# CelestineAngla/BundleAdjustment.jl

Hardware: AMD Instinct MI355X
Metric: LM iterations/sec on BAL venice-1778 (synthetic BAL-shaped), plus Jacobian Mnnz/sec (higher is better)
Workload: dtype f64; 1 GPU; venice-1778 shape: ncams=1778 npnts=993923 nobs=5001946, seed 20261004, lm.jl variant, LDL/None, facto_type f64, fixed 83 iterations, perm AMD; parallelism=points sharded over 1 rank(s), cameras replicated

## Files before the change

bundleadjustment.jl_amd/csrc/ba_dense_ldl.hip:

```cpp
#include "ba_internal.h"

#include <algorithm>
#include <atomic>
#include <cmath>
#include <cstdio>
#include <cstdlib>

namespace {

template <typename T>
struct RT;
template <>
struct RT<double> {
  typedef double v4 __attribute__((ext_vector_type(4)));
  typedef double v2 __attribute__((ext_vector_type(2)));
  static __device__ inline v4 mfma(double a, double b, v4 c) { return __builtin_amdgcn_mfma_f64_16x16x4f64(a, b, c, 0, 0, 0); }
  static __device__ inline int row(int lane, int reg) { return (lane >> 4) + 4 * reg; }
};
template <>
struct RT<float> {
  typedef float v4 __attribute__((ext_vector_type(4)));
  typedef float v2 __attribute__((ext_vector_type(2)));
  static __device__ inline v4 mfma(float a, float b, v4 c) { return __builtin_amdgcn_mfma_f32_16x16x4f32(a, b, c, 0, 0, 0); }
  static __device__ inline int row(int lane, int reg) { return 4 * (lane >> 4) + reg; }
// ... 1272 lines not shown
  matvec_t(Linv + (int64_t)k * NB * NB, zk);
  __syncthreads();
  if (tid < NB) xk[tid] = part[0][tid] + part[1][tid];
  __syncthreads();
  if (tkk >= 0) matvec_t(S + tkk * NB * NB, xk);
  else part[half][c] = 0;
  __syncthreads();
  if (tid < NB) {
    const T d = D[(int64_t)(k - 1) * NB + tid];
    zk[tid] = (y[(int64_t)(k - 1) * NB + tid] - d * (part[0][tid] + part[1][tid])) / d;
  }
  __syncthreads();
  matvec_t(Linv + (int64_t)(k - 1) * NB * NB, zk);
  __syncthreads();
  if (tid < NB) xk1[tid] = part[0][tid] + part[1][tid];
  __syncthreads();
  if (bid == 0) {
    if (tid < NB) {
      x[(int64_t)k * NB + tid] = xk[tid];
      x[(int64_t)(k - 1) * NB + tid] = xk1[tid];
    }
    return;
  }
  const T *Lkj = S + tkj * NB * NB, *Lk1j = S + tk1j * NB * NB;
  T s = 0;
  if (tkj >= 0 && tk1j >= 0) {
    for (int r = half * 64; r < half * 64 + 64; r++) s += Lkj[r * NB + c] * xk[r] + Lk1j[r * NB + c] * xk1[r];
  } else if (tkj >= 0) {
    for (int r = half * 64; r < half * 64 + 64; r++) s += Lkj[r * NB + c] * xk[r];
  } else if (tk1j >= 0) {
    for (int r = half * 64; r < half * 64 + 64; r++) s += Lk1j[r * NB + c] * xk1[r];
  }
  part[half][c] = s;
  __syncthreads();
  if (tid < NB) y[(int64_t)j * NB + tid] -= D[(int64_t)j * NB + tid] * (part[0][tid] + part[1][tid]);
}

template <typename T>
__global__ __launch_bounds__(256) void k_bwd_pair(const T *__restrict__ S, const int64_t *__restrict__ co, const T *__restrict__ Linv,
                                                   const T *__restrict__ D, T *__restrict__ y, T *__restrict__ x, int k,
                                                   const int *__restrict__ cols = nullptr) {
  bwd_pair_body<T>(S, co, Linv, D, y, x, k, cols, (int)blockIdx.x);
}
template <typename T>
__global__ __launch_bounds__(256) void k_bwd_pair2(const T *__restrict__ S, const int64_t *__restrict__ co, const T *__restrict__ Linv,
                                                    const T *__restrict__ D, T *__restrict__ y, T *__restrict__ x, int ka,
                                                    const int *__restrict__ cols_a, int na, int kc, const int *__restrict__ cols_c) {
  const bool second = (int)blockIdx.x >= na;
  bwd_pair_body<T>(S, co, Linv, D, y, x, second ? kc : ka, second ? cols_c : cols_a, (int)blockIdx.x - (second ? na : 0));
}


template <typename T>
__global__ __launch_bounds__(256) void k_fwd_step_multi(const T *__restrict__ S, const int64_t *__restrict__ co, const T *__restrict__ Linv,
                                                         T *__restrict__ b, T *__restrict__ y, int k, int64_t ld) {
  BA_VT
  __shared__ T yk[NB];
  const int tid = threadIdx.x, lane = tid & 63, wv = tid >> 6;
  const int i = k + blockIdx.x;
  const int64_t tik = blockIdx.x == 0 ? 0 : tix(co, i, k);
  if (tik < 0) return;
  b += (int64_t)blockIdx.y * ld;
  y += (int64_t)blockIdx.y * ld;
  const T *Lk = Linv + (int64_t)k * NB * NB;
  const d2 bk = *reinterpret_cast<const d2 *>(b + (int64_t)k * NB + 2 * lane);
  for (int rr = 0; rr < 32; rr++) {
    int row = wv * 32 + rr;
    d2 l = *reinterpret_cast<const d2 *>(Lk + row * NB + 2 * lane);
    T s = wsum(l.x * bk.x + l.y * bk.y);
    if (lane == 0) yk[row] = s;
  }
  __syncthreads();
  if (blockIdx.x == 0) {
    if (tid < NB) y[(int64_t)k * NB + tid] = yk[tid];
    return;
  }
  const T *Lik = S + tik * NB * NB;
  const T y0 = yk[2 * lane], y1 = yk[2 * lane + 1];
  for (int rr = 0; rr < 32; rr++) {
    int row = wv * 32 + rr;
    d2 l = *reinterpret_cast<const d2 *>(Lik + row * NB + 2 * lane);
    T s = wsum(l.x * y0 + l.y * y1);
    if (lane == 0) b[(int64_t)i * NB + row] -= s;
  }
}

template <typename T>
__global__ __launch_bounds__(256) void k_bwd_step_multi(const T *__restrict__ S, const int64_t *__restrict__ co, const T *__restrict__ Linv,
                                                         const T *__restrict__ D, T *__restrict__ y, T *__restrict__ x, int k, int64_t ld) {
  __shared__ T zk[NB], xk[NB], part[2][NB];
  const int tid = threadIdx.x;
  const int c = tid & (NB - 1), half = tid >> 7;
  const int j = (int)blockIdx.x - 1;
  const int64_t tkj = blockIdx.x == 0 ? 0 : tix(co, k, j);
  if (tkj < 0) return;
  y += (int64_t)blockIdx.y * ld;
  x += (int64_t)blockIdx.y * ld;
  if (tid < NB) zk[tid] = y[(int64_t)k * NB + tid] / D[(int64_t)k * NB + tid];
  __syncthreads();
  {
    const T *Lk = Linv + (int64_t)k * NB * NB;
    T s = 0;
    for (int r = half * 64; r < half * 64 + 64; r++) s += Lk[r * NB + c] * zk[r];
    part[half][c] = s;
  }
  __syncthreads();
  if (tid < NB) xk[tid] = part[0][tid] + part[1][tid];
  __syncthreads();
  if (blockIdx.x == 0) {
    if (tid < NB) x[(int64_t)k * NB + tid] = xk[tid];
    return;
  }
  const T *Lkj = S + tkj * NB * NB;
  T s = 0;
  for (int r = half * 64; r < half * 64 + 64; r++) s += Lkj[r * NB + c] * xk[r];
  part[half][c] = s;
  __syncthreads();
  if (tid < NB) y[(int64_t)j * NB + tid] -= D[(int64_t)j * NB + tid] * (part[0][tid] + part[1][tid]);
}

}

int64_t dense_ldl_tiles_doubles(int64_t n_unpadded) {
  int64_t nt = (n_unpadded + NB - 1) / NB;
  if (nt < 1) nt = 1;
  return nt * (nt + 1) / 2 * NB * NB;
}

template <typename T>
static int set_kernel_attrs() {
  static std::atomic<bool> g_attr_done{false};
  if (g_attr_done.load()) return BA_OK;
  BA_HIP_CHECK(hipFuncSetAttribute(reinterpret_cast<const void *>(k_ldl_diag<T>),
                                   hipFuncAttributeMaxDynamicSharedMemorySize, (int)(DIAG_LDS_ELEMS * sizeof(T))));
  BA_HIP_CHECK(hipFuncSetAttribute(reinterpret_cast<const void *>(k_ldl_update<T, 1>),
                                   hipFuncAttributeMaxDynamicSharedMemorySize, (int)gemm_priv_lds_bytes<T>()));
  BA_HIP_CHECK(hipFuncSetAttribute(reinterpret_cast<const void *>(k_ldl_pairdiag<T, true>),
                                   hipFuncAttributeMaxDynamicSharedMemorySize, (int)(DIAG_LDS_ELEMS * sizeof(T))));
  BA_HIP_CHECK(hipFuncSetAttribute(reinterpret_cast<const void *>(k_ldl_pairdiag<T, false>),
                                   hipFuncAttributeMaxDynamicSharedMemorySize, (int)(DIAG_LDS_ELEMS * sizeof(T))));
  BA_HIP_CHECK(hipFuncSetAttribute(reinterpret_cast<const void *>(k_ldl_pairtrsm<T, true>),
                                   hipFuncAttributeMaxDynamicSharedMemorySize, (int)(PT_LDS_ELEMS * sizeof(T))));
  BA_HIP_CHECK(hipFuncSetAttribute(reinterpret_cast<const void *>(k_ldl_pairtrsm<T, false>),
                                   hipFuncAttributeMaxDynamicSharedMemorySize, (int)(PT_LDS_ELEMS * sizeof(T))));
  BA_HIP_CHECK(hipFuncSetAttribute(reinterpret_cast<const void *>(k_ldl_update_rs<T>),
                                   hipFuncAttributeMaxDynamicSharedMemorySize, (int)(RS_LDS_ELEMS * sizeof(T))));
  BA_HIP_CHECK(hipFuncSetAttribute(reinterpret_cast<const void *>(k_ldl_update2<T>), hipFuncAttributeMaxDynamicSharedMemorySize,
                                   (int)gemm_priv_lds_bytes<T>()));
  BA_HIP_CHECK(hipFuncSetAttribute(reinterpret_cast<const void *>(k_ldl_diag2<T>), hipFuncAttributeMaxDynamicSharedMemorySize,
                                   (int)(DIAG_LDS_ELEMS * sizeof(T))));
  BA_HIP_CHECK(hipFuncSetAttribute(reinterpret_cast<const void *>(k_ldl_update_part2<T>), hipFuncAttributeMaxDynamicSharedMemorySize,
                                   (int)part_lds_bytes<T>()));
  BA_HIP_CHECK(hipFuncSetAttribute(reinterpret_cast<const void *>(k_ldl_update_part<T>),
                                   hipFuncAttributeMaxDynamicSharedMemorySize, (int)part_lds_bytes<T>()));
  BA_HIP_CHECK(hipFuncSetAttribute(reinterpret_cast<const void *>(k_ldl_update<T, 1, true>),
                                   hipFuncAttributeMaxDynamicSharedMemorySize, (int)gemm_priv_lds_bytes<T>()));
  g_attr_done.store(true);
  return BA_OK;
}

void dense_ldl_layout(int64_t nt, int world, std::vector<int64_t> *col_off, std::vector<int64_t> *own_range) {
  col_off->assign((size_t)nt, 0);
  if (own_range) own_range->assign((size_t)world + 1, 0);
  int64_t off = 0;
  for (int r = 0; r < world; r++) {
    if (own_range) (*own_range)[(size_t)r] = off;
    for (int64_t q = r; 2 * q < nt; q += world)
      for (int64_t j = 2 * q; j < 2 * q + 2 && j < nt; j++) {
        (*col_off)[(size_t)j] = off;
        off += nt - j;
      }
  }
  if (own_range) (*own_range)[(size_t)world] = off;
}

template <typename T>
int dense_ldl_alloc(DenseLDLT<T> *w, int64_t n_unpadded, int world, int rank, bool lazy_S, bool own_only) {
  int64_t nt = (n_unpadded + NB - 1) / NB;
  if (nt < 1) nt = 1;
  w->n = nt * NB;
  w->nt = nt;
  w->world = world;
  w->rank = rank;
  dense_ldl_layout(nt, world, &w->h_glob_off, &w->own_range);
  w->h_col_tab.assign((size_t)nt + 1, 0);
  for (int64_t j = 0; j < nt; j++) w->hco()[j] = w->h_glob_off[(size_t)j];
  w->own_only = own_only && world > 1;
  w->s_tiles = nt * (nt + 1) / 2;
  if (w->own_only) {
    const int64_t base = w->own_range[(size_t)rank];
    for (int64_t j = 0; j < nt; j++)
      w->hco()[j] = ((j / 2) % world == rank) ? w->hco()[j] - base : BA_NO_TILE;
    w->s_tiles = std::max<int64_t>(1, w->own_range[(size_t)rank + 1] - base);
  }
  BA_CHECK(upload(w->col_tab, w->h_col_tab));
  w->col_off = w->col_tab + 1;
  w->h_own_cols.clear();
  w->h_own_pref.assign(1, 0);
  for (int64_t j = 0; j < nt; j++)
    if ((j / 2) % world == rank) {
      w->h_own_cols.push_back((int)j);
      w->h_own_pref.push_back(w->h_own_pref.back() + (nt - j));
    }
  BA_CHECK(upload(w->own_cols, w->h_own_cols, 1));
  BA_CHECK(upload(w->own_pref, w->h_own_pref));
  BA_CHECK(w->flag_sum.alloc(1));
  if (!lazy_S) BA_CHECK(dense_ldl_alloc_S(w));
  BA_CHECK(w->ev_chain.create(hipEventDisableTiming | hipEventReleaseToDevice));
  BA_CHECK(w->Linv.alloc(nt * NB * NB));
  BA_HIP_CHECK(hipMemset(w->Linv, 0, (size_t)nt * NB * NB * sizeof(T)));
  BA_HIP_CHECK(hipDeviceSynchronize());
  BA_CHECK(w->D.alloc(nt * NB * 2));
  BA_CHECK(w->flag.alloc(1));
  BA_CHECK(w->ready.alloc(nt));
  BA_CHECK(w->hoist.create(hipStreamNonBlocking));
  {
    int lo = 0, hi = 0;
    BA_HIP_CHECK(hipDeviceGetStreamPriorityRange(&lo, &hi));
    BA_CHECK(w->rest.create(hipStreamNonBlocking, lo));
  }
  BA_CHECK(w->ev_top.create(hipEventDisableTiming | hipEventReleaseToDevice));
  BA_CHECK(w->ev_dtop.create(hipEventDisableTiming));
  BA_CHECK(w->ev_dchain.create(hipEventDisableTiming));
  for (int q = 0; q < 2; q++) {
    BA_CHECK(w->ev_recv[q].create(hipEventDisableTiming));
    BA_CHECK(w->ev_upd[q].create(hipEventDisableTiming));
  }
  return set_kernel_attrs<T>();
}

template <typename T>
int dense_ldl_alloc_S(DenseLDLT<T> *w) {
  if (!w->S) BA_CHECK(w->S.alloc(w->s_tiles * NB * NB));
  if (!w->V) BA_CHECK(w->V.alloc(8 * w->nt * NB * NB));
  if (!w->Lb && w->own_only) BA_CHECK(w->Lb.alloc(4 * w->nt * NB * NB));
  if (!w->bpart && w->own_only) BA_CHECK(w->bpart.alloc(2 * w->nt * NB));
  return BA_OK;
}

struct PairRows {
  int k, c1, c2;
  const int *rows1, *rows2;
  const int *h_rows1;
  int row(int a) const { return h_rows1 ? h_rows1[a] : k + 1 + a; }
};

template <typename T>
static PairRows pair_rows(const DenseLDLT<T> *w, int q) {
  PairRows r = {2 * q, 0, 0, nullptr, nullptr, nullptr};
  if (const TilePattern *pat = w->pat) {
    const int l0 = pat->prow_ptr[(size_t)q];
    r.c1 = pat->prow_ptr[(size_t)q + 1] - l0;
    r.rows1 = w->prow + l0;
    r.rows2 = r.rows1 + 1;
    r.h_rows1 = pat->prow.data() + l0;
  } else {
    r.c1 = std::max(0, (int)w->nt - r.k - 1);
  }
  r.c2 = r.c1 > 0 ? r.c1 - 1 : 0;
  return r;
}

template <typename T>
static int launch_diag(ba_problem *p, DenseLDLT<T> *w, int k, hipStream_t st, const int *wait_ready = nullptr, bool clear_flag = false) {
  ProfScope ps(p, PC_LDL_DIAG, st);
  hipLaunchKernelGGL(k_ldl_diag<T>, dim3(1), dim3(DIAG_THREADS), DIAG_LDS_ELEMS * sizeof(T), st, w->S + tix(w->hco(), k, k) * NB * NB,
                     w->Linv + (int64_t)k * NB * NB, w->D + (int64_t)k * NB, w->flag, (unsigned long long *)nullptr,
// ... 544 lines not shown
    __syncthreads();
    matvec_t(S + tix(co, k + 1, k) * NB * NB, xk1);
    __syncthreads();
  }
  if (tid < NB) {
    T s = two ? red[0][tid] + red[1][tid] : (T)0;
    if (rows)
      for (int a = 0; a < nrows; a++) s += part[(int64_t)rows[a] * NB + tid];
    else
      for (int i = k + 2; i < nt; i++) s += part[(int64_t)i * NB + tid];
    z[tid] = y[(int64_t)k * NB + tid] / D[(int64_t)k * NB + tid] - s;
  }
  __syncthreads();
  matvec_t(Linv + (int64_t)k * NB * NB, z);
  __syncthreads();
  if (tid < NB) x[(int64_t)k * NB + tid] = red[0][tid] + red[1][tid];
}

template <typename T>
static int dense_ldl_bwd_dist(ba_problem *p, DenseLDLT<T> *w, T *d_b, hipStream_t st) {
  const int nt = (int)w->nt, P = w->world, me = w->rank;
  const T *y = w->D + (int64_t)nt * NB;
  const int last = ((nt - 1) / 2) * 2;
  for (int k = last; k >= 0; k -= 2) {
    const int owner = (k / 2) % P;
    const bool two = k + 1 < nt;
    if (owner == me) {
      const PairRows r = pair_rows(w, k / 2);
      if (r.c2 > 0) hipLaunchKernelGGL(k_bwd_col_part<T>, dim3(2 * r.c2), dim3(256), 0, st, w->S, w->col_off, d_b, w->bpart, k, nt, r.rows2);
      hipLaunchKernelGGL(k_bwd_col_final<T>, dim3(1), dim3(256), 0, st, w->S, w->col_off, w->Linv, w->D, y, w->bpart, d_b, k, nt, r.rows2,
                         r.c2);
      BA_HIP_CHECK(hipGetLastError());
    }
    BA_CHECK(comm_bcast(p, d_b + (int64_t)k * NB, (int64_t)(two ? 2 : 1) * NB * sizeof(T), owner, st));
  }
  return BA_OK;
}

template <typename T>
int dense_ldl_solve(ba_problem *p, DenseLDLT<T> *w, T *d_b, hipStream_t st, bool forward_done) {
  const int nt = (int)w->nt;
  T *y = w->D + (int64_t)nt * NB;
  ProfScope ps(p, PC_SOLVE, st);
  if (w->own_only && p->comm.active()) {
    if (!forward_done) {
      ba_set_error("per-rank ownership of S: the forward substitution rides along with the distributed factorisation");
      return BA_ERR_ARG;
    }
    return dense_ldl_bwd_dist(p, w, d_b, st);
  }
  if (!forward_done)
    for (int k = 0; k < nt; k++)
      hipLaunchKernelGGL(k_fwd_step<T>, dim3(nt - k), dim3(256), 0, st, w->S, w->col_off, w->Linv, d_b, y, k);
  if (w->sparse && !p->comm.active()) {
    const TilePattern *pat = w->pat;
    if (!forward_done) {
      ba_set_error("block-sparse reduced camera system: the forward substitution rides along with the factorisation");
      return BA_ERR_ARG;
    }
    const int npairs = (nt + 1) / 2;
    auto single = [&](int q) {
      const int k = 2 * q + 1;
      if (k >= nt) {
        const int c0 = pat->lcol_ptr[(size_t)(nt - 1)], c1 = pat->lcol_ptr[(size_t)nt];
        hipLaunchKernelGGL(k_bwd_step<T>, dim3(1 + (c1 - c0)), dim3(256), 0, st, w->S, w->col_off, w->Linv, w->D, y, d_b, nt - 1, w->lcol + c0);
      } else {
        const int c0 = pat->lpair_ptr[(size_t)q], c1 = pat->lpair_ptr[(size_t)q + 1];
        hipLaunchKernelGGL(k_bwd_pair<T>, dim3(1 + (c1 - c0)), dim3(256), 0, st, w->S, w->col_off, w->Linv, w->D, y, d_b, k, w->lpair + c0);
      }
    };
    int c_hi = pat->split + pat->b_clean;
    if (c_hi > 0 && 2 * c_hi - 1 >= nt) c_hi--;
    if (pat->split > 0 && c_hi > pat->split && !env_off("BA_SPARSE_TWO_RUNS") && !env_off("BA_SPARSE_BWD2")) {
      for (int q = npairs - 1; q >= c_hi; q--) single(q);
      const int both = std::min(pat->split, c_hi - pat->split);
      for (int i = 0; i < both; i++) {
        const int qa = pat->split - 1 - i, qc = c_hi - 1 - i;
        const int a0 = pat->lpair_ptr[(size_t)qa], a1 = pat->lpair_ptr[(size_t)qa + 1];
        const int c0 = pat->lpair_ptr[(size_t)qc], c1 = pat->lpair_ptr[(size_t)qc + 1];
        hipLaunchKernelGGL(k_bwd_pair2<T>, dim3(2 + (a1 - a0) + (c1 - c0)), dim3(256), 0, st, w->S, w->col_off, w->Linv, w->D, y, d_b,
                           2 * qa + 1, w->lpair + a0, 1 + (a1 - a0), 2 * qc + 1, w->lpair + c0);
      }
      for (int q = pat->split - 1 - both; q >= 0; q--) single(q);
      for (int q = c_hi - 1 - both; q >= pat->split; q--) single(q);
    } else {
      for (int q = npairs - 1; q >= 0; q--) single(q);
    }
    BA_HIP_CHECK(hipGetLastError());
    return BA_OK;
  }
  int k = nt - 1;
  for (; k >= 1; k -= 2)
    hipLaunchKernelGGL(k_bwd_pair<T>, dim3(k), dim3(256), 0, st, w->S, w->col_off, w->Linv, w->D, y, d_b, k);
  if (k == 0)
    hipLaunchKernelGGL(k_bwd_step<T>, dim3(1), dim3(256), 0, st, w->S, w->col_off, w->Linv, w->D, y, d_b, 0);
  BA_HIP_CHECK(hipGetLastError());
  return BA_OK;
}

template <typename T>
int dense_ldl_solve_multi(ba_problem *p, DenseLDLT<T> *w, T *d_B, int64_t ld, int m, T *d_y, hipStream_t st) {
  const int nt = (int)w->nt;
  if (m <= 0) return BA_OK;
  if (w->own_only || p->comm.active() || ld < w->n) {
    ba_set_error("multi-right-hand-side solve: one rank holding all of S, column stride >= the padded order");
    return BA_ERR_ARG;
  }
  ProfScope ps(p, PC_SHARED_SWEEP, st);
  for (int k = 0; k < nt; k++)
    hipLaunchKernelGGL(k_fwd_step_multi<T>, dim3(nt - k, m), dim3(256), 0, st, w->S, w->col_off, w->Linv, d_B, d_y, k, ld);
  for (int k = nt - 1; k >= 0; k--)
    hipLaunchKernelGGL(k_bwd_step_multi<T>, dim3(1 + k, m), dim3(256), 0, st, w->S, w->col_off, w->Linv, w->D, d_y, d_B, k, ld);
  BA_HIP_CHECK(hipGetLastError());
  return BA_OK;
}

template <typename T>
static int dense_solve_host(int device, int64_t n, const double *a_lower_rowmajor, const double *b, double *x,
                            double *factor_ms) {
  if (n <= 0 || !a_lower_rowmajor || !b || !x) {
    ba_set_error("ba_dense_ldl_solve: bad argument");
    return BA_ERR_ARG;
  }
  BA_HIP_CHECK(hipSetDevice(device));
  ba_problem tmp;
  DenseLDLT<T> w;
  BA_CHECK(dense_ldl_alloc<T>(&w, n));
  const int64_t npad = w.n;
  std::vector<T> tiles((size_t)dense_ldl_tiles_doubles(n), (T)0);
  for (int64_t i = 0; i < npad; i++) {
    int64_t ti = i / NB;
    for (int64_t j = 0; j <= i; j++) {
      int64_t tj = j / NB;
      double v = (i < n) ? a_lower_rowmajor[i * n + j] : (i == j ? 1.0 : 0.0);
      tiles[(size_t)((tix(w.hco(), ti, tj) * NB + (i - ti * NB)) * NB + (j - tj * NB))] = (T)v;
    }
  }
  std::vector<T> bb((size_t)npad, (T)0);
  for (int64_t i = 0; i < n; i++) bb[(size_t)i] = (T)b[i];
  DevBuf<T> d_b;
  hipStream_t st = nullptr;
  HipEvent e0, e1;
  BA_CHECK(d_b.alloc(npad));
  BA_HIP_CHECK(hipMemcpy(w.S, tiles.data(), tiles.size() * sizeof(T), hipMemcpyHostToDevice));
  BA_HIP_CHECK(hipMemcpy(d_b, bb.data(), (size_t)npad * sizeof(T), hipMemcpyHostToDevice));
  BA_CHECK(e0.create());
  BA_CHECK(e1.create());
  int rc = BA_OK, zp = 0;
  for (int attempt = 0; attempt < 2; attempt++) {
    BA_HIP_CHECK(hipEventRecord(e0, st));
    rc = dense_ldl_factor<T>(&tmp, &w, st, d_b);
    BA_HIP_CHECK(hipEventRecord(e1, st));
    if (rc == BA_OK) rc = dense_ldl_solve<T>(&tmp, &w, d_b, st, true);
    BA_HIP_CHECK(hipMemcpy(&zp, w.flag, sizeof(int), hipMemcpyDeviceToHost));
    BA_HIP_CHECK(hipDeviceSynchronize());
    if (zp != 2 || w.hoist_disabled) break;
    w.hoist_disabled = true;
    BA_HIP_CHECK(hipMemcpy(w.S, tiles.data(), tiles.size() * sizeof(T), hipMemcpyHostToDevice));
    BA_HIP_CHECK(hipMemcpy(d_b, bb.data(), (size_t)npad * sizeof(T), hipMemcpyHostToDevice));
  }
  float ms = 0;
  BA_HIP_CHECK(hipEventElapsedTime(&ms, e0, e1));
  if (factor_ms) *factor_ms = ms;
  BA_HIP_CHECK(hipMemcpy(bb.data(), d_b, (size_t)npad * sizeof(T), hipMemcpyDeviceToHost));
  for (int64_t i = 0; i < n; i++) x[i] = (double)bb[(size_t)i];
  if (rc == BA_OK && zp) {
    ba_set_error("dense LDL': exactly zero pivot");
    return BA_ERR_ZERO_PIVOT;
  }
  return rc;
}

extern "C" int ba_dense_ldl_solve(int device, int64_t n, const double *a_lower_rowmajor, const double *b, double *x,
                                  double *factor_ms) {
  return dense_solve_host<double>(device, n, a_lower_rowmajor, b, x, factor_ms);
}

extern "C" int ba_dense_ldl_solve_f32(int device, int64_t n, const double *a_lower_rowmajor, const double *b, double *x,
                                      double *factor_ms) {
  return dense_solve_host<float>(device, n, a_lower_rowmajor, b, x, factor_ms);
}

extern "C" int ba_dense_ldl_solve_multi(int device, int64_t n, const double *a_lower_rowmajor, int nrhs, const double *B, double *X,
                                        double *factor_ms) {
  if (n <= 0 || nrhs <= 0 || !a_lower_rowmajor || !B || !X) {
    ba_set_error("ba_dense_ldl_solve_multi: bad argument");
    return BA_ERR_ARG;
  }
  BA_HIP_CHECK(hipSetDevice(device));
  ba_problem tmp;
  DenseLDL w;
  BA_CHECK(dense_ldl_alloc<double>(&w, n));
  const int64_t npad = w.n;
  std::vector<double> tiles((size_t)dense_ldl_tiles_doubles(n), 0.0);
  for (int64_t i = 0; i < npad; i++) {
    const int64_t ti = i / NB;
    for (int64_t j = 0; j <= i; j++) {
      const int64_t tj = j / NB;
      const double v = (i < n) ? a_lower_rowmajor[i * n + j] : (i == j ? 1.0 : 0.0);
      tiles[(size_t)((tix(w.hco(), ti, tj) * NB + (i - ti * NB)) * NB + (j - tj * NB))] = v;
    }
  }
  std::vector<double> bb((size_t)(npad * nrhs), 0.0);
  for (int c = 0; c < nrhs; c++)
    for (int64_t i = 0; i < n; i++) bb[(size_t)(c * npad + i)] = B[(int64_t)c * n + i];
  DevBuf<double> d_b, d_y;
  hipStream_t st = nullptr;
  HipEvent e0, e1;
  BA_CHECK(d_b.alloc(npad * nrhs));
  BA_CHECK(d_y.alloc(npad * nrhs));
// ... 43 lines not shown
```

bundleadjustment.jl_amd/csrc/ba_internal.h:

```cpp
#pragma once
#include <hip/hip_runtime.h>
#include <stdint.h>
#include <stdlib.h>
#include <string>
#include <vector>

#include "../../include/ba_hip.h"
#include "ba_order.h"

void ba_set_error(const char *fmt, ...);

#define BA_HIP_CHECK(expr)                                                                          \
  do {                                                                                              \
    hipError_t _e = (expr);                                                                         \
    if (_e != hipSuccess) {                                                                         \
      ba_set_error("%s:%d: %s -> %s", __FILE__, __LINE__, #expr, hipGetErrorString(_e));            \
      return BA_ERR_HIP;                                                                            \
    }                                                                                               \
  } while (0)

#define BA_CHECK(expr)            \
  do {                            \
    int _rc = (expr);             \
    if (_rc != BA_OK) return _rc; \
// ... 135 lines not shown
  PC_LDL_SYRK,
  PC_LDL_UPDATE,
  PC_LDL_UPDATE_RS,
  PC_SOLVE,
  PC_BACKSUB,
  PC_TRIAL,
  PC_REDUCE,
  PC_COMM,
  PC_ROBUST,
  PC_FIXED,
  PC_COV_INV,
  PC_COV_CAMS,
  PC_COV_POINTS,
  PC_PRIOR,
  PC_SHARED_BORDER,
  PC_SHARED_SWEEP,
  PC_SHARED_SMALL,
  PC_COUNT
};
extern const char *const kProfNames[PC_COUNT];

struct ProfSlot {
  double ms = 0;
  int64_t calls = 0;
};

template <typename T>
struct DenseLDLT {
  int64_t n = 0, nt = 0;
  DevBuf<T> S;
  DevBuf<T> V;
  T *vpanel(int slot, int j, int run = 0) { return V + (int64_t)(4 * run + 2 * slot + j) * nt * NB * NB; }
  DevBuf<T> Linv;
  DevBuf<T> D;
  int64_t *col_off = nullptr;
  std::vector<int64_t> h_col_tab;
  DevBuf<int64_t> col_tab;
  const int64_t *hco() const { return h_col_tab.data() + 1; }
  int64_t *hco() { return h_col_tab.data() + 1; }
  std::vector<int64_t> own_range;
  int world = 1, rank = 0;
  std::vector<int> h_own_cols;
  std::vector<int64_t> h_own_pref;
  DevBuf<int> own_cols;
  DevBuf<int64_t> own_pref;
  DevBuf<double> flag_sum;
  DevBuf<int> flag;
  DevBuf<int> ready;
  HipStream hoist;
  HipStream rest;
  HipEvent ev_top;
  bool hoist_disabled = false;
  bool hoisting = false;
  HipEvent ev_chain;
  HipEvent ev_recv[2], ev_upd[2];
  bool own_only = false;
  int64_t s_tiles = 0;
  std::vector<int64_t> h_glob_off;
  DevBuf<T> Lb, bpart;
  T *L_of(const T *v) { return Lb + (v - V); }
  bool sparse = false;
  const TilePattern *pat = nullptr;
  DevBuf<int> prow, lcol, lpair;
  std::vector<int64_t> h_col_cnt;
  std::vector<int> h_upd_ptr, h_upd_lead;
  DevBuf<int2> upd_ij, own_tiles;
  HipEvent ev_dtop, ev_dchain;
};
typedef DenseLDLT<double> DenseLDL;
constexpr int HOIST_MIN_TILES = 32;
constexpr int HOIST_MAX_TILES = 224;

struct BaComm {
  int rank = 0, world = 1;
  ba_comm_fn hook = nullptr;
  void *hook_ctx = nullptr;
  void *nccl = nullptr;
  int64_t calls = 0, bytes = 0;
  int64_t op_calls[BA_COMM_OPS] = {}, op_bytes[BA_COMM_OPS] = {};
  bool active() const { return hook != nullptr || nccl != nullptr; }
};

void lm_free(ba_problem *p);

struct PriorSet {
  int64_t n = 0;
  std::vector<int> h_idx;
  std::vector<double> h_mu, h_info;
  DevBuf<int> idx;
  DevBuf<double> mu, info;
};
enum { PRI_PNT = 0, PRI_CAM, PRI_CTR, PRI_KINDS };

struct ba_problem {
  int device = 0;
  HipStream stream;
  int64_t ncams = 0, npnts = 0, nobs = 0;
  DevBuf<int> cam0, pnt0;
  DevBuf<double> pt2d;
  DevBuf<float> pt2d_f32;
  DevBuf<int> pt_ptr, pt_obs;
  DevBuf<int> cam_ptr, cam_obs;
  bool point_sorted = false;
  std::vector<int> h_cam0, h_pnt0, h_pt_ptr, h_pt_obs;
  DevBuf<char> scratch[4];
  size_t scratch_bytes[4] = {0, 0, 0, 0};
// ... 90 lines not shown
```

bundleadjustment.jl_amd/csrc/ba_lm.hip:

```cpp
#include <algorithm>
#include <chrono>
#include <cmath>
#include <cstdio>
#include <cstring>

#include "ba_internal.h"
#include "ba_lm_internal.h"

namespace {

double wall() {
  using namespace std::chrono;
  return duration<double>(steady_clock::now().time_since_epoch()).count();
}

enum { SH_RSQ = 0, SH_GP, SH_X_P, SH_RTSQ, SH_RSQ_TRIAL, SH_MODEL, SH_DELTA_P, SH_COUNT = 8 };
constexpr int SH_LIN_COUNT = 3, SH_TRIAL_FIRST = 4, SH_TRIAL_COUNT = 3;
enum { RP_DELTA_C = 0, RP_X_C, RP_GC, RP_COUNT = 8 };
static_assert(SH_RSQ == 0 && SH_X_P == SH_LIN_COUNT - 1 && SH_RTSQ == SH_LIN_COUNT, "linearisation slots: one run from slot 0");
static_assert(SH_RSQ_TRIAL == SH_TRIAL_FIRST && SH_DELTA_P == SH_TRIAL_FIRST + SH_TRIAL_COUNT - 1, "trial slots: one run");
static_assert(SH_RTSQ < SH_TRIAL_FIRST && SH_TRIAL_FIRST + SH_TRIAL_COUNT <= SH_COUNT, "the two runs do not overlap");

int build_tasks(ba_problem *p, SchurTasks *T, const std::vector<int> &pos) {
  const int64_t ncams = p->ncams, npnts = p->npnts;
// ... 911 lines not shown
    jobs.add(w->delta, 3 * p->npnts, w->scal, SH_DELTA_P);
    jobs.add(w->delta + 3 * p->npnts, w->n, w->scal_rep, RP_DELTA_C);
    if (p->pri_on()) jobs.add_sum(p->pri_model(), p->pri_total(), w->scal, SH_MODEL, true);
    BA_CHECK(launch_sumsq_multi(p, &jobs, w->partial_multi, st));
  }
  return BA_OK;
}

static int trial_point(ba_problem *p, LMWork *w, bool with_delta, bool recorded, hipStream_t st) {
  BA_CHECK(launch_axpy(p, w->nvar, w->x, w->delta, w->x_trial, st));
  if (w->mode.xf32) {
    BA_CHECK(launch_convert(w->x_trial, w->xf, w->nvar, st));
    BA_CHECK(launch_convert(w->xf, w->x_trial, w->nvar, st));
    BA_CHECK(launch_residual_f32(p, w->xf, w->rf, st));
    BA_CHECK(launch_convert(w->rf, w->r_trial, w->nequ, st));
  } else {
    BA_CHECK(launch_residual_f64(p, w->x_trial, w->r_trial, st));
  }
  const bool robust = p->loss != BA_LOSS_LINEAR;
  if (!with_delta && p->pri_on()) {
    ba_set_error("trial point of a rescaled step with priors (internal error: the line search is refused with priors)");
    return BA_ERR_ARG;
  }
  if (!with_delta && !robust) return launch_sumsq(p, w->nequ, w->r_trial, w->partial, w->scal, SH_RSQ_TRIAL, st);
  SumsqJobs jobs;
  if (with_delta) {
    jobs.add(w->delta, 3 * p->npnts, w->scal, SH_DELTA_P);
    jobs.add(w->delta + 3 * p->npnts, w->n, w->scal_rep, RP_DELTA_C);
  }
  if (robust) jobs.add_robust(w->r_trial, p->nobs, w->scal, SH_RSQ_TRIAL, p->loss, p->loss_scale * p->loss_scale);
  else jobs.add(w->r_trial, w->nequ, w->scal, SH_RSQ_TRIAL);
  if (p->pri_on()) {
    BA_CHECK(launch_prior_step(p, w->delta, w->x_trial, st));
    jobs.add_sum(p->pri_model(), p->pri_total(), w->scal, SH_MODEL, true);
    jobs.add_sum(p->pri_cost_trial(), p->pri_total(), w->scal, SH_RSQ_TRIAL, true);
  }
  if (recorded) jobs.publish(w->scal, SH_COUNT, w->h_sh, w->scal_rep, RP_COUNT, w->h_rp, w->pivot_flag(), w->h_flag);
  return launch_sumsq_multi(p, &jobs, w->partial_multi, st);
}

static int pivot_flag_error(int h, const char *zero_pivot_msg = "reduced camera system: exactly zero pivot (SQDException in the reference)") {
  if (h == 2) {
    ba_set_error("dense factorisation: a hoisted diagonal tile never became ready (internal scheduling error)");
    return BA_ERR_HIP;
  }
  if (h) {
    ba_set_error("%s", zero_pivot_msg);
    return BA_ERR_ZERO_PIVOT;
  }
  return BA_OK;
}

static bool hoist_gave_up(LMWork *w) {
  if (*w->h_flag != 2 || (w->ldl.hoist_disabled && w->ldl32.hoist_disabled)) return false;
  w->ldl.hoist_disabled = w->ldl32.hoist_disabled = true;
  return true;
}

template <typename F>
static int with_hoist_retry(LMWork *w, F body) {
  BA_CHECK(body());
  if (hoist_gave_up(w)) BA_CHECK(body());
  return BA_OK;
}

static RecordedFor recorded_for(ba_problem *p, LMWork *w) {
  const StepMode &m = w->mode;
  const int bits = m.normalize + 4 * (m.facto_f32 ? 1 : 0) + 8 * (m.xf32 ? 1 : 0) + 16 * p->loss + 128 * (p->fix_ncam > 0 ? 1 : 0) +
                   256 * (p->fix_npnt > 0 ? 1 : 0);
  RecordedFor f;
  f.bits = bits;
  f.loss_scale = p->loss != BA_LOSS_LINEAR ? p->loss_scale : 1.0;
  f.d_fix_cam = p->d_fix_cam;
  f.d_fix_pnt = p->d_fix_pnt;
  if (p->pri_on()) {
    for (int k = 0; k < PRI_KINDS; k++) {
      const PriorSet &q = p->pri[k];
      f.n_pri[k] = q.n;
      if (q.n > 0) f.d_pri[k][0] = q.idx, f.d_pri[k][1] = q.mu, f.d_pri[k][2] = q.info;
    }
    f.d_pri_work[0] = p->pri_d, f.d_pri_work[1] = p->pri_H, f.d_pri_work[2] = p->pri_val;
  }
  return f;
}
static bool recorded_current(ba_problem *p, LMWork *w) { return w->rec.made_for == recorded_for(p, w); }

static bool graphs_allowed(ba_problem *p, LMWork *w) {
  if (w->rec.off || p->prof_on || p->comm.active() || w->mode.f16 || w->mode.pcg || p->grp_on()) return false;
  if (w->ldl.nt >= HOIST_MIN_TILES + 2 && !w->use_pattern) return false;
  return !env_off("BA_LM_GRAPH");
}

template <typename F>
static int record_graph(hipStream_t st, HipGraphExec *out, F body) {
  HipGraph g;
  BA_HIP_CHECK(hipStreamBeginCapture(st, hipStreamCaptureModeRelaxed));
  const int rc = body();
  const hipError_t e = hipStreamEndCapture(st, g.out());
  BA_CHECK(rc);
  BA_HIP_CHECK(e);
  BA_HIP_CHECK(hipGraphInstantiate(out->out(), g, nullptr, nullptr, 0));
  return BA_OK;
}

template <typename F>
static int replay(LMWork *w, HipGraphExec *g, hipStream_t st, F body) {
  if (!*g && record_graph(st, g, body) != BA_OK) {
    (void)hipGetLastError();
    g->reset();
    w->rec.off = true;
    return BA_OK;
  }
  BA_HIP_CHECK(hipGraphLaunch(*g, st));
  BA_HIP_CHECK(hipStreamSynchronize(st));
  return BA_OK;
}

static int trial_step(ba_problem *p, LMWork *w, double lambda, hipStream_t st) {
  auto launches = [&](double lam, bool recorded) -> int {
    BA_CHECK(linear_step(p, w, lam, recorded, st));
    BA_CHECK(step_scalars(p, w, st, -1.0, true));
    return trial_point(p, w, true, recorded, st);
  };
  if (graphs_allowed(p, w)) {
    if (!recorded_current(p, w)) {
      w->rec = RecordedSequences();
      w->rec.made_for = recorded_for(p, w);
    }
    if (w->mode.facto_f32) BA_CHECK(ensure_f32(w));
    *w->h_lambda = lambda;
    BA_CHECK(replay(w, &w->rec.step[w->parity], st, [&]() -> int { return launches(1.0, true); }));
    if (!w->rec.off) return BA_OK;
  }
  return with_hoist_retry(w, [&]() -> int {
    BA_CHECK(launches(lambda, false));
    BA_CHECK(comm_allreduce(p, w->scal + SH_TRIAL_FIRST, SH_TRIAL_COUNT, st));
    BA_HIP_CHECK(hipMemcpyAsync(w->h_flag, w->pivot_flag(), sizeof(int), hipMemcpyDeviceToHost, st));
    return fetch_scalars(p, w, st);
  });
}

static int accept_refresh(ba_problem *p, LMWork *w, hipStream_t st) {
  if (graphs_allowed(p, w)) {
    BA_CHECK(replay(w, &w->rec.refresh[w->parity], st, [&]() -> int {
      return refresh_linearisation(p, w, false, true, st);
    }));
    if (!w->rec.off) return BA_OK;
  }
  BA_CHECK(refresh_linearisation(p, w, false, false, st));
  return fetch_scalars(p, w, st);
}

static bool can_prefetch_trial(ba_problem *p, LMWork *w) {
  if (env_off("BA_LM_PREFETCH") || !graphs_allowed(p, w)) return false;
  return recorded_current(p, w) && w->rec.step[w->parity] && w->rec.refresh[w->parity];
}
static int accept_refresh_and_trial(LMWork *w, double lambda, hipStream_t st) {
  BA_HIP_CHECK(hipGraphLaunch(w->rec.refresh[w->parity], st));
  *w->h_lambda = lambda;
  BA_HIP_CHECK(hipGraphLaunch(w->rec.step[w->parity], st));
  BA_HIP_CHECK(hipStreamSynchronize(st));
  return BA_OK;
}

static int lm_step_impl(ba_problem *p, const double *x, double lambda, double *delta, double *half_sq_model,
                        double *jtr, bool facto_f32, bool pcg = false, double tol = 0, int max_iter = 0, int *cg_iters = nullptr) {
  if (!p || !x || !delta) {
    ba_set_error("ba_lm_step: null argument");
    return BA_ERR_ARG;
  }
  if (p->pri_on() && p->comm.active()) {
    ba_set_error("ba_lm_step: priors (ba_lm_set_priors) are not supported on a handle with a communicator");
    return BA_ERR_ARG;
  }
  if (p->grp_on()) {
    if (p->comm.active()) {
      ba_set_error("ba_lm_step: shared intrinsics (ba_lm_set_shared_intrinsics) are not supported on a handle with a communicator");
      return BA_ERR_ARG;
    }
    if (facto_f32) {
      ba_set_error("ba_lm_step_f32: shared intrinsics (ba_lm_set_shared_intrinsics) are not supported with facto_type = Float32");
      return BA_ERR_ARG;
    }
    BA_CHECK(shared_check(p, x + 3 * p->npnts, "ba_lm_step"));
  }
// ... 378 lines not shown
    const TS n = ts::f32(std::sqrt(sumsq));
    return ts::div(ts::mul(n, n), ts::f32(2));
  };

  memset(stats, 0, sizeof *stats);
  stats->status = BA_ST_UNKNOWN;
  double *h_sh = w->h_sh, *h_rp = w->h_rp;

  BA_HIP_CHECK(hipMemcpyAsync(w->x, x_inout, (size_t)w->nvar * sizeof(double), x_on_device ? hipMemcpyDeviceToDevice : hipMemcpyHostToDevice, st));
  if (xf32) {
    BA_CHECK(launch_convert(w->x, w->xf, w->nvar, st));
    BA_CHECK(launch_convert(w->xf, w->x, w->nvar, st));
  }
  BA_CHECK(refresh_linearisation(p, w, true, false, st));
  BA_CHECK(fetch_scalars(p, w, st));
  stats->n_residual++;
  stats->n_jacobian++;
  const bool robust = p->loss != BA_LOSS_LINEAR;
  TS norm_r = norm_of(h_sh[SH_RSQ], W);
  TS obj = robust ? half_of(h_sh[SH_RSQ]) : ts::div(ts::mul(norm_r, norm_r), T_(2));
  TS norm_Jtr = norm_of(h_sh[SH_GP] + h_rp[RP_GC], W);
  TS norm_x = norm_of(h_sh[SH_X_P] + h_rp[RP_X_C], W);
  bool all_fixed = false;
  if (p->fix_ncam == 9 * p->ncams) {
    double free_pts = (double)(p->npnts - p->fix_npnt);
    if (p->comm.active()) {
      BA_HIP_CHECK(hipMemcpyAsync(w->partial, &free_pts, sizeof(double), hipMemcpyHostToDevice, st));
      BA_CHECK(comm_allreduce(p, w->partial, 1, st));
      BA_HIP_CHECK(hipMemcpyAsync(&free_pts, w->partial, sizeof(double), hipMemcpyDeviceToHost, st));
      BA_HIP_CHECK(hipStreamSynchronize(st));
    }
    all_fixed = free_pts == 0;
  }
  if (all_fixed) norm_Jtr = T_(0);
  if (V && !all_fixed) {
    lambda = ts::max(lambda, ts::div(ts::f64(1e10), norm_Jtr));
    lambda = T_(lambda.v);
  }

  TS norm_delta = T_(0), dr2 = T_(0), ared = T_(0), pred = T_(0);
  const TS eps_first = ts::add(atol, ts::mul(rtol, norm_Jtr));
  TS old_obj = obj;
  bool small_step = false, first_order = all_fixed || norm_Jtr.v < eps_first.v, small_residual = norm_r.v < restol.v;
  bool small_obj_change = false, fail2 = false;
  int iter = 0;
  bool tired = iter > ite_max;
  bool accepted = false, have_trial = false;
  int rc = BA_OK;
  const double t_loop = wall();

  while (!(small_step || first_order || small_residual || small_obj_change || tired || fail2)) {
    if (V) iter++;
    if (!V && cb) cb(cb_ctx, iter, obj.v, ts::sub(old_obj, obj).v, norm_Jtr.v, lambda.v, norm_delta.v, dr2.v, accepted);
    if (have_trial) have_trial = false;
    else if ((rc = trial_step(p, w, lambda.v, st)) != BA_OK) break;
    stats->n_factor++;
    stats->n_residual++;
    if ((rc = pivot_flag_error(*w->h_flag)) != BA_OK) break;
    dr2 = half_of(h_sh[SH_MODEL]);
    const TS pred_r = ts::f64(0.5 * h_sh[SH_RTSQ] - 0.5 * h_sh[SH_MODEL]);
    if (robust) dr2 = ts::sub(obj, pred_r);
    TS obj_suiv = half_of(h_sh[SH_RSQ_TRIAL]);
    TS norm_rsuiv = norm_of(h_sh[SH_RSQ_TRIAL], W);
    if (!V) iter++;
    int delta_w = (xf32 && !(V && o->normalize == 2 && lambda.w == 64)) ? 32 : 64;

    bool step_accepted;
    int ntimes = 0;
    if (V) {
      pred = robust ? pred_r : ts::sub(obj, dr2);
      ared = ts::sub(obj, obj_suiv);
      step_accepted = ared.v >= 1e-4 * pred.v;
      double c_r = w->cr0();
      while (linesearch && !step_accepted && ntimes < 4) {
        if (!facto_qr) c_r = (c_r + 1.0) / delta_d.v;
        if (delta_d.w == 64) delta_w = 64;
        if ((rc = launch_scale_scalar(p, w->nvar, w->delta, 1.0 / delta_d.v, st)) != BA_OK) break;
        if ((rc = step_scalars(p, w, st, c_r)) != BA_OK) break;
        if ((rc = trial_point(p, w, false, false, st)) != BA_OK) break;
        stats->n_residual++;
        if ((rc = comm_allreduce(p, w->scal + SH_TRIAL_FIRST, SH_TRIAL_COUNT, st)) != BA_OK) break;
        if ((rc = fetch_scalars(p, w, st)) != BA_OK) break;
        dr2 = half_of(h_sh[SH_MODEL]);
        obj_suiv = half_of(h_sh[SH_RSQ_TRIAL]);
        norm_rsuiv = norm_of(h_sh[SH_RSQ_TRIAL], W);
        pred = ts::sub(obj, dr2);
        ared = ts::sub(obj, obj_suiv);
        step_accepted = ared.v >= 1e-4 * pred.v;
        ntimes++;
      }
      if (rc != BA_OK) break;
    } else {
      step_accepted = ts::sub(obj_suiv, obj).v < 1e-4 * (robust ? -pred_r.v : ts::sub(dr2, obj).v);
    }
    accepted = step_accepted;
    const TS nd = norm_of(h_sh[SH_DELTA_P] + h_rp[RP_DELTA_C], delta_w);

    if (V) {
      norm_delta = nd;
      if (std::isnan(norm_delta.v)) {
        fail2 = true;
        continue;
      }
      const double rho = ts::div(ared, pred).v;
      if (cb) cb(cb_ctx, iter, obj.v, ts::sub(old_obj, obj).v, norm_Jtr.v, lambda.v, norm_delta.v, rho,
                 (step_accepted && dr2.v <= obj.v) ? 1 : 0);
      if (o->verbose)
        fprintf(stderr, "%6d %14.7e %10.2e %10.2e %10.2e %10.2e %10.2e %s\n", iter, obj.v, ts::sub(old_obj, obj).v, norm_Jtr.v,
// ... 80 lines not shown
```

Measured before the change: 27.86 LM iterations/s.

## Replace per-step backward substitution launches with a single persistent dataflow sweep kernel

Result: slower. 27.52 LM iterations/s (-1.2%).

```diff
diff --git a/bundleadjustment.jl_amd/csrc/ba_dense_ldl.hip b/bundleadjustment.jl_amd/csrc/ba_dense_ldl.hip
--- a/bundleadjustment.jl_amd/csrc/ba_dense_ldl.hip
+++ b/bundleadjustment.jl_amd/csrc/ba_dense_ldl.hip
@@ -1348,6 +1348,214 @@
 
 
 template <typename T>
+__device__ __forceinline__ T bwd_fma(T a, T b, T c);
+template <>
+__device__ __forceinline__ double bwd_fma<double>(double a, double b, double c) { return __builtin_fma(a, b, c); }
+template <>
+__device__ __forceinline__ float bwd_fma<float>(float a, float b, float c) { return __builtin_fmaf(a, b, c); }
+template <typename T>
+__device__ __forceinline__ T bwd_mul(T a, T b) {
+#pragma clang fp contract(off)
+  return a * b;
+}
+template <typename T>
+__device__ __forceinline__ T bwd_add(T a, T b) {
+#pragma clang fp contract(off)
+  return a + b;
+}
+template <typename T, int STRIDE>
+__device__ __forceinline__ T bwd_dot1(const T *M, const T *v) {
+  constexpr int UNR = STRIDE == 1 ? 64 : 32, FUSED = sizeof(T) == 4 ? 52 : 64;
+  T s = 0;
+#pragma unroll UNR
+  for (int r = 0; r < 64; r++) s = r < FUSED ? bwd_fma<T>(M[r * STRIDE], v[r], s) : bwd_add<T>(s, bwd_mul<T>(M[r * STRIDE], v[r]));
+  return s;
+}
+template <typename T>
+__device__ __forceinline__ T bwd_dot2(const T *Ma, const T *va, const T *Mb, const T *vb) {
+  T s = 0;
+#pragma unroll 16
+  for (int r = 0; r < 64; r++) s = bwd_add<T>(s, bwd_fma<T>(Ma[r * NB], va[r], bwd_mul<T>(Mb[r * NB], vb[r])));
+  return s;
+}
+constexpr int BWD_SWEEP_THREADS = 512;
+constexpr int BWD_SWEEP_MAX_UNITS = 1024;
+constexpr unsigned BWD_SWEEP_POLLS = 1u << 18;
+struct BwdUnit {
+  int k, k1;
+};
+__host__ __device__ inline BwdUnit bwd_unit(int u, int nt, bool from_top) {
+  BwdUnit r;
+  if (from_top) {
+    r.k = 2 * u + 1 - (nt & 1);
+    r.k1 = r.k - 1;
+  } else {
+    r.k = 2 * u + 1;
+    r.k1 = 2 * u;
+    if (r.k >= nt) r.k = 2 * u, r.k1 = -1;
+  }
+  return r;
+}
+template <typename T>
+size_t bwd_sweep_lds_bytes(int nu) {
+  const size_t need = (size_t)(NB * NB + 9 * NB) * sizeof(T) + 16 * ((size_t)nu + 1);
+  return std::max(need, (size_t)84 * 1024);
+}
+__device__ __forceinline__ void st_agent(double *p, double v) {
+  __hip_atomic_store(reinterpret_cast<unsigned long long *>(p), (unsigned long long)__double_as_longlong(v), __ATOMIC_RELAXED,
+                     __HIP_MEMORY_SCOPE_AGENT);
+}
+__device__ __forceinline__ void st_agent(float *p, float v) {
+  __hip_atomic_store(reinterpret_cast<unsigned *>(p), __float_as_uint(v), __ATOMIC_RELAXED, __HIP_MEMORY_SCOPE_AGENT);
+}
+__device__ __forceinline__ double ld_agent(const double *p) {
+  return __longlong_as_double((long long)__hip_atomic_load(reinterpret_cast<const unsigned long long *>(p), __ATOMIC_RELAXED,
+                                                           __HIP_MEMORY_SCOPE_AGENT));
+}
+__device__ __forceinline__ float ld_agent(const float *p) {
+  return __uint_as_float(__hip_atomic_load(reinterpret_cast<const unsigned *>(p), __ATOMIC_RELAXED, __HIP_MEMORY_SCOPE_AGENT));
+}
+
+template <typename T>
+__global__ __launch_bounds__(BWD_SWEEP_THREADS) void k_bwd_sweep(const T *__restrict__ S, const int64_t *__restrict__ co,
+                                                                  const T *__restrict__ Linv, const T *__restrict__ D,
+                                                                  const T *__restrict__ y, T *x, int nt, int from_top, unsigned *prog,
+                                                                  int *flag, unsigned max_polls) {
+  extern __shared__ __attribute__((aligned(16))) unsigned char smraw[];
+  T *tile = reinterpret_cast<T *>(smraw);
+  T *yv = tile + NB * NB;
+  T *xs = yv + 2 * NB;
+  T *zk = xs + 2 * NB;
+  T *part = zk + NB;
+  int4 *tt = reinterpret_cast<int4 *>(part + 4 * NB);
+  int *okf = reinterpret_cast<int *>(tt + (nt + 1) / 2);
+  const int tid = threadIdx.x, g = tid >> 8, t = tid & 255, c = t & (NB - 1), half = t >> 7;
+  const int nu = (nt + 1) / 2, u = nu - 1 - (int)blockIdx.x;
+  const BwdUnit me = bwd_unit(u, nt, from_top != 0);
+  const int k = me.k, k1 = me.k1;
+  const bool pair = k1 >= 0;
+  const int o = half * 64 * NB + c, vo = half * 64;
+  constexpr int TILE_LINES = NB * NB * (int)sizeof(T) / 128, PF = 4 * TILE_LINES / BWD_SWEEP_THREADS;
+  auto tile_of = [&](int i, int j) -> int {
+    if (i < 0 || j < 0) return -1;
+    const int64_t q = tix(co, i, j);
+    return q < 0 ? -1 : (int)q;
+  };
+  for (int v = u + 1 + tid; v < nu; v += BWD_SWEEP_THREADS) {
+    const BwdUnit w = bwd_unit(v, nt, from_top != 0);
+    tt[v] = make_int4(tile_of(w.k, k), tile_of(w.k1, k), tile_of(w.k, k1), tile_of(w.k1, k1));
+  }
+  const int tkk = pair ? tile_of(k, k1) : -1;
+  T hold[64];
+  {
+    const T *src = g == 0 ? Linv + (int64_t)k * NB * NB : (tkk >= 0 ? S + (int64_t)tkk * NB * NB : nullptr);
+#pragma unroll
+    for (int r = 0; r < 64; r++) hold[r] = src ? src[o + r * NB] : (T)0;
+  }
+  if (pair) {
+    const uint4 *src = reinterpret_cast<const uint4 *>(Linv + (int64_t)k1 * NB * NB);
+    uint4 *dst = reinterpret_cast<uint4 *>(tile);
+    for (int i = tid; i < NB * NB * (int)sizeof(T) / 16; i += BWD_SWEEP_THREADS) dst[i] = src[i];
+  }
+  const int jc = g == 0 ? k : k1;
+  T dj = 0;
+  if (t < NB && jc >= 0) {
+    dj = D[(int64_t)jc * NB + t];
+    yv[g * NB + t] = y[(int64_t)jc * NB + t];
+  }
+  __syncthreads();
+  unsigned pf[PF];
+  auto prefetch = [&](int v) {
+#pragma unroll
+    for (int i = 0; i < PF; i++) {
+      const int line = tid + i * BWD_SWEEP_THREADS, q = line / TILE_LINES;
+      int tl = -1;
+      if (v > u) {
+        const int4 e = tt[v];
+        tl = q == 0 ? e.x : q == 1 ? e.y : q == 2 ? e.z : e.w;
+      }
+      pf[i] = tl >= 0 ? *reinterpret_cast<const unsigned *>(reinterpret_cast<const char *>(S + (int64_t)tl * NB * NB) + (size_t)(line % TILE_LINES) * 128) : 0u;
+    }
+  };
+  auto prefetch_done = [&]() {
+#pragma unroll
+    for (int i = 0; i < PF; i++) asm volatile("" ::"v"(pf[i]));
+  };
+  prefetch(nu - 1);
+  prefetch_done();
+  bool alive = true;
+  for (int v = nu - 1; v > u; v--) {
+    const int4 e = tt[v];
+    prefetch(v - 1);
+    if ((e.x & e.y & e.z & e.w) < 0 && e.x < 0 && e.y < 0 && e.z < 0 && e.w < 0) {
+      prefetch_done();
+      continue;
+    }
+    if (tid == 0) {
+      bool ok = false;
+      for (unsigned n = 0;; n++) {
+        if (__hip_atomic_load(prog + v, __ATOMIC_RELAXED, __HIP_MEMORY_SCOPE_AGENT) != 0u) {
+          ok = true;
+          break;
+        }
+        if (n >= max_polls) break;
+        if ((n & 63u) == 0u && __hip_atomic_load(flag, __ATOMIC_RELAXED, __HIP_MEMORY_SCOPE_AGENT) == 2) break;
+        __builtin_amdgcn_s_sleep(2);
+      }
+      if (!ok) __hip_atomic_store(flag, 2, __ATOMIC_RELAXED, __HIP_MEMORY_SCOPE_AGENT);
+      *okf = ok;
+    }
+    __syncthreads();
+    if (!*okf) {
+      alive = false;
+      break;
+    }
+    const BwdUnit w = bwd_unit(v, nt, from_top != 0);
+    if (tid < NB) xs[tid] = ld_agent(x + (int64_t)w.k * NB + tid);
+    else if (tid < 2 * NB && w.k1 >= 0) xs[tid] = ld_agent(x + (int64_t)w.k1 * NB + (tid - NB));
+    __syncthreads();
+    const int ta = g == 0 ? e.x : e.z, tb = g == 0 ? e.y : e.w;
+    const T *La = S + (int64_t)ta * NB * NB + o, *Lb = S + (int64_t)tb * NB * NB + o;
+    T s = 0;
+    if (ta >= 0 && tb >= 0) s = bwd_dot2<T>(La, xs + vo, Lb, xs + NB + vo);
+    else if (ta >= 0) s = bwd_dot1<T, NB>(La, xs + vo);
+    else if (tb >= 0) s = bwd_dot1<T, NB>(Lb, xs + NB + vo);
+    part[(g * 2 + half) * NB + c] = s;
+    prefetch_done();
+    __syncthreads();
+    if (t < NB && (ta >= 0 || tb >= 0)) yv[g * NB + t] = bwd_fma<T>(-dj, bwd_add<T>(part[(g * 2) * NB + t], part[(g * 2 + 1) * NB + t]), yv[g * NB + t]);
+  }
+  if (!alive) return;
+  __syncthreads();
+  T xk_own = 0, xk1_own = 0;
+  if (tid < NB) zk[tid] = yv[tid] / dj;
+  __syncthreads();
+  if (g == 0) part[half * NB + c] = bwd_dot1<T, 1>(hold, zk + vo);
+  __syncthreads();
+  if (tid < NB) xs[tid] = xk_own = part[tid] + part[NB + tid];
+  __syncthreads();
+  if (pair) {
+    if (g == 1) part[(2 + half) * NB + c] = tkk >= 0 ? bwd_dot1<T, 1>(hold, xs + vo) : (T)0;
+    __syncthreads();
+    if (tid < NB) {
+      const T d = D[(int64_t)k1 * NB + tid];
+      zk[tid] = bwd_fma<T>(-d, bwd_add<T>(part[2 * NB + tid], part[3 * NB + tid]), yv[NB + tid]) / d;
+    }
+    __syncthreads();
+    if (g == 0) part[half * NB + c] = bwd_dot1<T, NB>(tile + o, zk + vo);
+    __syncthreads();
+    if (tid < NB) xk1_own = part[tid] + part[NB + tid];
+  }
+  if (tid < NB) {
+    st_agent(x + (int64_t)k * NB + tid, xk_own);
+    if (pair) st_agent(x + (int64_t)k1 * NB + tid, xk1_own);
+  }
+  asm volatile("s_waitcnt vmcnt(0)" ::: "memory");
+  __syncthreads();
+  if (tid == 0) __hip_atomic_store(prog + u, 1u, __ATOMIC_RELAXED, __HIP_MEMORY_SCOPE_AGENT);
+}
+
+template <typename T>
 __global__ __launch_bounds__(256) void k_fwd_step_multi(const T *__restrict__ S, const int64_t *__restrict__ co, const T *__restrict__ Linv,
                                                          T *__restrict__ b, T *__restrict__ y, int k, int64_t ld) {
   BA_VT
@@ -1451,6 +1659,8 @@
                                    hipFuncAttributeMaxDynamicSharedMemorySize, (int)part_lds_bytes<T>()));
   BA_HIP_CHECK(hipFuncSetAttribute(reinterpret_cast<const void *>(k_ldl_update<T, 1, true>),
                                    hipFuncAttributeMaxDynamicSharedMemorySize, (int)gemm_priv_lds_bytes<T>()));
+  BA_HIP_CHECK(hipFuncSetAttribute(reinterpret_cast<const void *>(k_bwd_sweep<T>), hipFuncAttributeMaxDynamicSharedMemorySize,
+                                   (int)bwd_sweep_lds_bytes<T>(BWD_SWEEP_MAX_UNITS)));
   g_attr_done.store(true);
   return BA_OK;
 }
@@ -1509,6 +1719,12 @@
   BA_CHECK(w->D.alloc(nt * NB * 2));
   BA_CHECK(w->flag.alloc(1));
   BA_CHECK(w->ready.alloc(nt));
+  BA_CHECK(w->bwd_prog.alloc(((nt + 1) / 2 + 3) / 4 * 4));
+  {
+    int dev = 0;
+    BA_HIP_CHECK(hipGetDevice(&dev));
+    BA_HIP_CHECK(hipDeviceGetAttribute(&w->n_cu, hipDeviceAttributeMultiprocessorCount, dev));
+  }
   BA_CHECK(w->hoist.create(hipStreamNonBlocking));
   {
     int lo = 0, hi = 0;
@@ -2159,12 +2375,22 @@
   if (!forward_done)
     for (int k = 0; k < nt; k++)
       hipLaunchKernelGGL(k_fwd_step<T>, dim3(nt - k), dim3(256), 0, st, w->S, w->col_off, w->Linv, d_b, y, k);
-  if (w->sparse && !p->comm.active()) {
+  const bool sparse = w->sparse && !p->comm.active();
+  if (sparse && !forward_done) {
+    ba_set_error("block-sparse reduced camera system: the forward substitution rides along with the factorisation");
+    return BA_ERR_ARG;
+  }
+  const int nu = (nt + 1) / 2;
+  if (!p->comm.active() && !w->bwd_disabled && nu <= w->n_cu && nu <= BWD_SWEEP_MAX_UNITS && env_int("BA_LDL_BWD_CHAIN", 0) == 0) {
+    const unsigned polls = (unsigned)std::max(0, env_int("BA_LDL_BWD_POLLS", (int)BWD_SWEEP_POLLS));
+    BA_HIP_CHECK(hipMemsetAsync(w->bwd_prog, 0, (size_t)((nu + 3) / 4 * 4) * sizeof(unsigned), st));
+    hipLaunchKernelGGL(k_bwd_sweep<T>, dim3(nu), dim3(BWD_SWEEP_THREADS), bwd_sweep_lds_bytes<T>(nu), st, w->S, w->col_off, w->Linv, w->D, y,
+                       d_b, nt, sparse ? 0 : 1, w->bwd_prog, w->flag, polls);
+    BA_HIP_CHECK(hipGetLastError());
+    return BA_OK;
+  }
+  if (sparse) {
     const TilePattern *pat = w->pat;
-    if (!forward_done) {
-      ba_set_error("block-sparse reduced camera system: the forward substitution rides along with the factorisation");
-      return BA_ERR_ARG;
-    }
     const int npairs = (nt + 1) / 2;
     auto single = [&](int q) {
       const int k = 2 * q + 1;
@@ -2261,8 +2487,8 @@
     if (rc == BA_OK) rc = dense_ldl_solve<T>(&tmp, &w, d_b, st, true);
     BA_HIP_CHECK(hipMemcpy(&zp, w.flag, sizeof(int), hipMemcpyDeviceToHost));
     BA_HIP_CHECK(hipDeviceSynchronize());
-    if (zp != 2 || w.hoist_disabled) break;
-    w.hoist_disabled = true;
+    if (zp != 2 || (w.hoist_disabled && w.bwd_disabled)) break;
+    w.hoist_disabled = w.bwd_disabled = true;
     BA_HIP_CHECK(hipMemcpy(w.S, tiles.data(), tiles.size() * sizeof(T), hipMemcpyHostToDevice));
     BA_HIP_CHECK(hipMemcpy(d_b, bb.data(), (size_t)npad * sizeof(T), hipMemcpyHostToDevice));
   }
diff --git a/bundleadjustment.jl_amd/csrc/ba_internal.h b/bundleadjustment.jl_amd/csrc/ba_internal.h
--- a/bundleadjustment.jl_amd/csrc/ba_internal.h
+++ b/bundleadjustment.jl_amd/csrc/ba_internal.h
@@ -211,6 +211,9 @@
   HipEvent ev_top;
   bool hoist_disabled = false;
   bool hoisting = false;
+  DevBuf<unsigned> bwd_prog;
+  int n_cu = 0;
+  bool bwd_disabled = false;
   HipEvent ev_chain;
   HipEvent ev_recv[2], ev_upd[2];
   bool own_only = false;
diff --git a/bundleadjustment.jl_amd/csrc/ba_lm.hip b/bundleadjustment.jl_amd/csrc/ba_lm.hip
--- a/bundleadjustment.jl_amd/csrc/ba_lm.hip
+++ b/bundleadjustment.jl_amd/csrc/ba_lm.hip
@@ -987,8 +987,8 @@
 }
 
 static bool hoist_gave_up(LMWork *w) {
-  if (*w->h_flag != 2 || (w->ldl.hoist_disabled && w->ldl32.hoist_disabled)) return false;
-  w->ldl.hoist_disabled = w->ldl32.hoist_disabled = true;
+  if (*w->h_flag != 2 || (w->ldl.hoist_disabled && w->ldl32.hoist_disabled && w->ldl.bwd_disabled && w->ldl32.bwd_disabled)) return false;
+  w->ldl.hoist_disabled = w->ldl32.hoist_disabled = w->ldl.bwd_disabled = w->ldl32.bwd_disabled = true;
   return true;
 }
 
@@ -1026,6 +1026,13 @@
   return !env_off("BA_LM_GRAPH");
 }
 
+static bool recorded_gave_up(ba_problem *p, LMWork *w) {
+  if (!hoist_gave_up(w)) return false;
+  w->rec = RecordedSequences();
+  w->rec.made_for = recorded_for(p, w);
+  return true;
+}
+
 template <typename F>
 static int record_graph(hipStream_t st, HipGraphExec *out, F body) {
   HipGraph g;
@@ -1065,7 +1072,7 @@
     if (w->mode.facto_f32) BA_CHECK(ensure_f32(w));
     *w->h_lambda = lambda;
     BA_CHECK(replay(w, &w->rec.step[w->parity], st, [&]() -> int { return launches(1.0, true); }));
-    if (!w->rec.off) return BA_OK;
+    if (!w->rec.off && !recorded_gave_up(p, w)) return BA_OK;
   }
   return with_hoist_retry(w, [&]() -> int {
     BA_CHECK(launches(lambda, false));
@@ -1550,8 +1557,10 @@
   while (!(small_step || first_order || small_residual || small_obj_change || tired || fail2)) {
     if (V) iter++;
     if (!V && cb) cb(cb_ctx, iter, obj.v, ts::sub(old_obj, obj).v, norm_Jtr.v, lambda.v, norm_delta.v, dr2.v, accepted);
-    if (have_trial) have_trial = false;
-    else if ((rc = trial_step(p, w, lambda.v, st)) != BA_OK) break;
+    if (have_trial) {
+      have_trial = false;
+      if (recorded_gave_up(p, w) && (rc = trial_step(p, w, lambda.v, st)) != BA_OK) break;
+    } else if ((rc = trial_step(p, w, lambda.v, st)) != BA_OK) break;
     stats->n_factor++;
     stats->n_residual++;
     if ((rc = pivot_flag_error(*w->h_flag)) != BA_OK) break;
```
